# yikaiw/Vidu4D

Hardware: AMD Instinct MI355X
Metric: train images/sec (fwd+bwd raster) @200k surfels, 512^2 (higher is better)
Workload: dtype f32

## Files before the change

include/vidu4d_surfel.h:

```cpp
#ifndef VIDU4D_SURFEL_H_INCLUDED
#define VIDU4D_SURFEL_H_INCLUDED

#include <stddef.h>
#include <stdint.h>

#ifdef __cplusplus
extern "C" {
#endif

#define VIDU4D_OK 0
#define VIDU4D_E_INVALID (-1)
#define VIDU4D_E_BUFFER (-2)
#define VIDU4D_E_HIP (-3)
#define VIDU4D_E_UNSUPPORTED (-4)

#define VIDU4D_SURFEL_ABI 21
int vidu4d_surfel_abi_version(void);
const char* vidu4d_last_error(void);

size_t vidu4d_surfel_geom_bytes(int P);
size_t vidu4d_surfel_image_bytes(int width, int height);
size_t vidu4d_surfel_binning_bytes(int64_t capacity );
size_t vidu4d_surfel_backward_workspace_bytes(int P);

// ... 16 lines not shown
    const float* transMat_precomp;
    const float* viewmatrix;
    const float* projmatrix;
    const float* campos;
    float* out_color;
    float* out_others;
    int32_t* radii;
    void* geom_buffer;
    size_t geom_bytes;
    void* image_buffer;
    size_t image_bytes;
    int segment_split;
    uint32_t* depth_used;
    int frames;
    const float* frame_viewmatrix[8];
    const float* frame_campos[8];
    float frame_tan_fovx[8];
    float frame_tan_fovy[8];
    const float* sh_dc;
    const float* sh_rest;
    int raw_params;
    int aux_planes;
    int assume_unsaturated;
    int long_list_sort;
    int debug_flags;
    int max_list_hint;
} Vidu4dSurfelForwardArgs;
#define VIDU4D_AUX_ALPHA 0x02
#define VIDU4D_AUX_GEOM 0x1F
#define VIDU4D_DEBUG_NO_CULL 1
#define VIDU4D_DEBUG_WHOLE_TILE_BACKWARD 2
#define VIDU4D_DEBUG_POSITION_ORDER 8
#define VIDU4D_DEBUG_SERIAL_REPAIR 4
#define VIDU4D_SCHED_PAIR(K) (((K) & 15) << 12)
#define VIDU4D_SCHED_XCD_BLOCK(B) (((B) & 15) << 8)
#define VIDU4D_SURFEL_MAX_FRAMES 8
size_t vidu4d_surfel_image_bytes_frames(int width, int height, int frames);

int vidu4d_surfel_forward_plan(const Vidu4dSurfelForwardArgs* args, void* stream);
int vidu4d_surfel_num_rendered(const Vidu4dSurfelForwardArgs* args, void* stream, int64_t* num_rendered);
int vidu4d_surfel_forward_run(const Vidu4dSurfelForwardArgs* args, void* binning_buffer, size_t binning_bytes,
                              int64_t capacity, void* stream);

typedef struct Vidu4dSurfelBackwardArgs {
    int P, D, M;
    int width, height;
    float tan_fovx, tan_fovy;
    float scale_modifier;
    int debug;
    const float* background;
    const float* means3D;
    const int32_t* radii;
    const float* shs;
    const float* colors_precomp;
    const float* scales;
    const float* rotations;
    const float* transMat_precomp;
    const float* viewmatrix;
    const float* projmatrix;
    const float* campos;
    const float* dL_dout_color;
    const float* dL_dout_others;
    const void* geom_buffer;
    const void* binning_buffer;
    int64_t binning_capacity;
    const void* image_buffer;
// ... 248 lines not shown
```

vidu4d_amd/_C.py:

```python
from __future__ import annotations

import contextlib
import ctypes as C
import math
import os
import threading

import torch

from . import _lib

_EXACT = os.environ.get("VIDU4D_SURFEL_EXACT", "0") == "1"
_SPLIT = os.environ.get("VIDU4D_SURFEL_SPLIT", "auto")
SPLIT_AUTO_LEN = int(os.environ.get("VIDU4D_SURFEL_SPLIT_AUTO_LEN", "2048"))
SPLIT_AUTO_TILES_PER_CU = float(os.environ.get("VIDU4D_SURFEL_SPLIT_AUTO_TILES_PER_CU",
                                               "1.25" if int(os.environ.get("VIDU4D_SURFEL_PAIR", "6")) > 0 else "2.0"))
SEG_LEN = int(os.environ.get("VIDU4D_SEG_LEN", "512"))
MSD_SORT_FROM = int(os.environ.get("VIDU4D_MSD_SORT_FROM", "10000"))
_SPEC = os.environ.get("VIDU4D_SURFEL_SPEC", "1") == "1"
_SPEC_GEOM = os.environ.get("VIDU4D_SURFEL_SPEC_GEOM", "0") == "1"
DEBUG_FLAGS = ((_lib.DEBUG_NO_CULL if os.environ.get("VIDU4D_SURFEL_NO_CULL", "0") == "1" else 0) |
               (_lib.DEBUG_WHOLE_TILE_BACKWARD if os.environ.get("VIDU4D_SURFEL_WHOLE_TILE_BWD", "0") == "1" else 0) |
               (_lib.DEBUG_SERIAL_REPAIR if os.environ.get("VIDU4D_SURFEL_SERIAL_REPAIR", "0") == "1" else 0) |
               (_lib.DEBUG_POSITION_ORDER if os.environ.get("VIDU4D_SURFEL_POSITION_ORDER", "0") == "1" else 0))
XCD_BLOCK = int(os.environ.get("VIDU4D_SURFEL_XCD_BLOCK", "0"))
PAIR_K = int(os.environ.get("VIDU4D_SURFEL_PAIR", "6"))
_cu_count: dict = {}


class RasterContext:

    def __init__(self, scope=None):
        self.scope = scope
        self.deferred = False
        self.graph_mode = False
        self.graph_headers = None
        self.pending: list = []
        self.grad_out: dict = {}
        self.grad_written = None
        self.debug_flags = None
        self.xcd_block = None
        self.pair_k = None
        self.walk_counters = None
        self.capacity_hint: dict = {}
        self.depth_hint: dict = {}
        self.len_hint: dict = {}
        self.long_tiles_hint: dict = {}
        self.unlimited: dict = {}
        self.depth_stat: dict = {}
        self.pinned: dict = {}

    def __enter__(self):
        _stack().append(self)
        return self

    def __exit__(self, *exc):
        _stack().pop()
# ... 493 lines not shown
```

vidu4d_amd/_lib.py:

```python
from __future__ import annotations

import ctypes as C
import os

_HERE = os.path.dirname(os.path.abspath(__file__))
LIB_PATH = os.path.join(_HERE, "csrc", "libvidu4d_surfel.so")

ABI_VERSION = 21


class ForwardArgs(C.Structure):
    _fields_ = [
        ("P", C.c_int), ("D", C.c_int), ("M", C.c_int), ("width", C.c_int), ("height", C.c_int),
        ("tan_fovx", C.c_float), ("tan_fovy", C.c_float), ("scale_modifier", C.c_float),
        ("prefiltered", C.c_int), ("debug", C.c_int),
        ("background", C.c_void_p), ("means3D", C.c_void_p), ("shs", C.c_void_p), ("colors_precomp", C.c_void_p),
        ("opacities", C.c_void_p), ("scales", C.c_void_p), ("rotations", C.c_void_p),
        ("transMat_precomp", C.c_void_p), ("viewmatrix", C.c_void_p), ("projmatrix", C.c_void_p),
        ("campos", C.c_void_p), ("out_color", C.c_void_p), ("out_others", C.c_void_p), ("radii", C.c_void_p),
        ("geom_buffer", C.c_void_p), ("geom_bytes", C.c_size_t), ("image_buffer", C.c_void_p),
        ("image_bytes", C.c_size_t), ("segment_split", C.c_int), ("depth_used", C.c_void_p),
        ("frames", C.c_int), ("frame_viewmatrix", C.c_void_p * 8), ("frame_campos", C.c_void_p * 8),
        ("frame_tan_fovx", C.c_float * 8), ("frame_tan_fovy", C.c_float * 8),
        ("sh_dc", C.c_void_p), ("sh_rest", C.c_void_p), ("raw_params", C.c_int), ("aux_planes", C.c_int),
# ... 23 lines not shown
                ("src_v", C.c_void_p), ("dst_v", C.c_void_p), ("width", C.c_int)]


class SkinFieldArgs(C.Structure):
    _fields_ = [("N", C.c_int), ("B", C.c_int), ("W", C.c_int), ("D", C.c_int)] + [
        (n, C.c_void_p) for n in ("xyz", "bone_A", "bone_c", "w_in", "b_in", "w_hid", "b_hid", "w_out", "b_out", "xbT",
                                  "rawT", "g_xbT", "g_rawT", "g_xyz", "relu_masks", "packed_fwd", "packed_bwd", "h_store",
                                  "g_store", "gx_store")] + [("h_store_rows", C.c_int)]


LOSS_MAX_FRAMES, LOSS_BLOCKS, LOSS_SUMS_FLOATS = 32, 1024, 32


class Stage3LossArgs(C.Structure):
    _fields_ = [("M", C.c_int), ("H", C.c_int), ("W", C.c_int), ("color", C.c_void_p * LOSS_MAX_FRAMES),
                ("allmap", C.c_void_p * LOSS_MAX_FRAMES), ("bkgd", C.c_void_p), ("rgb", C.c_void_p),
                ("mask", C.c_void_p), ("vis2d", C.c_void_p), ("det", C.c_void_p), ("lambda_dssim", C.c_float),
                ("rgb_wt", C.c_float), ("mask_wt", C.c_float), ("dist_wt", C.c_float), ("sums", C.c_void_p),
                ("partials", C.c_void_p), ("losses", C.c_void_p), ("plane_stride", C.c_int64),
                ("normal_wt", C.c_float), ("depth_ratio", C.c_float), ("rays_d", C.c_void_p * LOSS_MAX_FRAMES),
                ("rays_o", C.c_void_p * LOSS_MAX_FRAMES), ("view3x3", C.c_void_p * LOSS_MAX_FRAMES),
                ("surf_normal", C.c_void_p * LOSS_MAX_FRAMES), ("surf_depth", C.c_void_p)]


class Stage3LossGrads(C.Structure):
    _fields_ = [("g_color", C.c_void_p * LOSS_MAX_FRAMES), ("g_allmap", C.c_void_p * LOSS_MAX_FRAMES),
                ("g_bkgd", C.c_void_p), ("g_surf_normal", C.c_void_p * LOSS_MAX_FRAMES)]


SKIN_FIELD = dict(width=64, in_max=96, out_max=32, max_hidden=4)
AUX_ALPHA = 0x02
AUX_GEOM = 0x1F
DEBUG_NO_CULL, DEBUG_WHOLE_TILE_BACKWARD, DEBUG_SERIAL_REPAIR, DEBUG_POSITION_ORDER = 1, 2, 4, 8



def sched_pair(k: int) -> int:
    return (int(k) & 15) << 12


def sched_xcd_block(block: int) -> int:
    return (int(block) & 15) << 8


BLEND_STATS = 11
ADAM_MAX_TENSORS = 8
ADAMW_MAX_TENSORS = 32
CONTRACT_MAX_JOBS = 4
COPY_MAX_JOBS = 8
CLIP_MAX_TENSORS = 96
CLIP_WORKSPACE_FLOATS = 1056
DENSIFY_MAX_ATTRS = 8


class BackwardArgs(C.Structure):
    _fields_ = [
        ("P", C.c_int), ("D", C.c_int), ("M", C.c_int), ("width", C.c_int), ("height", C.c_int),
        ("tan_fovx", C.c_float), ("tan_fovy", C.c_float), ("scale_modifier", C.c_float), ("debug", C.c_int),
        ("background", C.c_void_p), ("means3D", C.c_void_p), ("radii", C.c_void_p), ("shs", C.c_void_p),
        ("colors_precomp", C.c_void_p), ("scales", C.c_void_p), ("rotations", C.c_void_p),
        ("transMat_precomp", C.c_void_p), ("viewmatrix", C.c_void_p), ("projmatrix", C.c_void_p),
        ("campos", C.c_void_p), ("dL_dout_color", C.c_void_p), ("dL_dout_others", C.c_void_p),
        ("geom_buffer", C.c_void_p), ("binning_buffer", C.c_void_p), ("binning_capacity", C.c_int64),
        ("image_buffer", C.c_void_p), ("workspace", C.c_void_p), ("workspace_bytes", C.c_size_t),
        ("dL_dmeans2D", C.c_void_p), ("dL_dcolors", C.c_void_p), ("dL_dopacity", C.c_void_p),
        ("dL_dmeans3D", C.c_void_p), ("dL_dtransMat", C.c_void_p), ("dL_dsh", C.c_void_p),
# ... 123 lines not shown
```

vidu4d_amd/csrc/binning.hip:

```cpp
#include <algorithm>

#include "surfel_state.h"
#include "wave_utils.h"

namespace surfel {

__global__ __launch_bounds__(1024) void tile_scan_kernel(GeomState g, ImageState img, int num_tiles)
{
    __shared__ uint32_t s_part[16];
    const int lane = threadIdx.x & 63, wave = threadIdx.x >> 6;
    uint32_t carry = 0;
    for (int base = 0; base < num_tiles; base += 1024) {
        const int t = base + threadIdx.x;
        uint32_t cnt[TILE_SLICES];
        uint32_t c = 0;
        if (t < num_tiles) {
            const uint4* p = reinterpret_cast<const uint4*>(img.tile_count + (size_t)t * TILE_SLICES);
#pragma unroll
            for (int k = 0; k < TILE_SLICES / 4; k++) {
                const uint4 v = p[k];
                cnt[4 * k] = v.x;
                cnt[4 * k + 1] = v.y;
                cnt[4 * k + 2] = v.z;
                cnt[4 * k + 3] = v.w;
// ... 395 lines not shown
            const size_t b = (size_t)(tile0 + y * cam.grid_x + x) * TILE_SLICES + slice;
            const uint32_t pos = img.tile_base[b] + atomicAdd(&img.tile_count[b], 1u);
            entries[pos] = entry;
        }
}

template <bool COMPACT>
__global__ __launch_bounds__(BIN_THREADS) void emit_keys_grouped_kernel(CameraParams cam, int P, int iters,
                                                                       const int32_t* radii, GeomState g,
                                                                       ImageState img, uint64_t* entries,
                                                                       int64_t capacity, ScheduleParams sp)
{
    extern __shared__ __attribute__((aligned(16))) uint32_t s_cur[];
    if (blockIdx.x == gridDim.x - 1) {
        tile_order(g, img, cam.grid_x * cam.grid_y * cam.frames, *reinterpret_cast<TileOrderShared*>(s_cur), sp);
        return;
    }
    if (blockIdx.x == 0 && threadIdx.x == 0) g.hdr->num_buckets = 0;
    if ((int64_t)g.hdr->num_rendered > capacity) {
        if (blockIdx.x == 0 && threadIdx.x == 0) g.hdr->overflow = 1;
        return;
    }
    const int frame_tiles = cam.grid_x * cam.grid_y, num_tiles = frame_tiles * cam.frames;
    const uint32_t* row = img.group_counts + (size_t)blockIdx.x * num_tiles;
    for (int t = threadIdx.x; t < num_tiles; t += BIN_THREADS) s_cur[t] = img.ranges[2 * t] + row[t];
    __syncthreads();
    const int first = blockIdx.x * BIN_THREADS * iters;
    for (int it = 0; it < iters; it++) {
        const int idx = first + it * BIN_THREADS + threadIdx.x;
        if (idx >= P) continue;
        int radius;
        float cx, cy, depth;
        if (COMPACT) {
            const float4 c = reinterpret_cast<const float4*>(g.colour)[idx];
            cx = c.x, cy = c.y, depth = c.z, radius = __float_as_int(c.w);
            if (radius <= 0) continue;
        } else {
            radius = radii[idx];
            if (radius <= 0) continue;
            const float4 q2 = reinterpret_cast<const float4*>(g.rec + (size_t)idx * REC_FLOATS)[2];
            const float4 q3 = reinterpret_cast<const float4*>(g.rec + (size_t)idx * REC_FLOATS)[3];
            cx = q2.y, cy = q2.z, depth = q3.w;
        }
        int x0, y0, x1, y1;
        tile_rect(cx, cy, radius, cam.grid_x, cam.grid_y, x0, y0, x1, y1);
        const uint64_t entry = ((uint64_t)__float_as_uint(depth) << 32) | (uint32_t)idx;
        uint32_t* cur = s_cur + (cam.frames > 1 ? (idx / cam.frame_surfels) * frame_tiles : 0);
        for (int y = y0; y < y1; y++)
            for (int x = x0; x < x1; x++) entries[atomicAdd(&cur[y * cam.grid_x + x], 1u)] = entry;
    }
}

void launch_emit_keys(const CameraParams& cam, int P, const int32_t* radii, const GeomState& g, const ImageState& img,
                      const BinState& b, int64_t capacity, bool grouped, const ScheduleParams& sp, hipStream_t stream)
{
    if (P <= 0 || capacity <= 0) {
        launch_tile_order(g, img, total_tiles(cam), sp, stream);
        return;
    }
    if (grouped) {
        auto kernel = preprocess_stages_records(total_tiles(cam)) ? &emit_keys_grouped_kernel<true> : &emit_keys_grouped_kernel<false>;
        const size_t lds = std::max((size_t)total_tiles(cam) * sizeof(uint32_t), sizeof(TileOrderShared));
        hipLaunchKernelGGL(kernel, dim3(bin_groups(P) + 1), dim3(BIN_THREADS), lds, stream,
                           cam, P, bin_iters(P), radii, g, img, b.entries, capacity, sp);
    } else {
        launch_tile_order(g, img, total_tiles(cam), sp, stream);
        hipLaunchKernelGGL(emit_keys_kernel, dim3(pre_blocks(P)), dim3(PRE_BLOCK), 0, stream, cam, P, radii, g, img,
// ... 324 lines not shown
```

vidu4d_amd/csrc/capi.hip:

```cpp
#include <stdarg.h>
#include <stdio.h>
#include <string.h>

#include <vector>

#include "../../include/vidu4d_surfel.h"
#include "../../include/vidu4d_surfel_diag.h"
#include "surfel_state.h"

using namespace surfel;

static thread_local char g_err[512] = "";

static int fail(int code, const char* fmt, ...)
{
    va_list ap;
    va_start(ap, fmt);
    vsnprintf(g_err, sizeof(g_err), fmt, ap);
    va_end(ap);
    return code;
}

#define HIP_TRY(expr)                                                                                  \
    do {                                                                                               \
// ... 189 lines not shown
    if (int rc = check_frames(a)) return rc;
    if (F == 1 && (!(a->tan_fovx > 0.f) || !(a->tan_fovy > 0.f))) return fail(VIDU4D_E_INVALID, "tan_fov must be > 0");
    if (!a->out_color || !a->out_others || !a->background) return fail(VIDU4D_E_INVALID, "output/background pointer is NULL");
    if (a->P > 0 && (!a->means3D || !a->opacities || !a->scales || !a->rotations || !a->radii ||
                     (F == 1 && (!a->viewmatrix || !a->campos))))
        return fail(VIDU4D_E_INVALID, "an input pointer is NULL");
    if (!a->geom_buffer || a->geom_bytes < vidu4d_surfel_geom_bytes(a->P * F)) return fail(VIDU4D_E_BUFFER, "geom_buffer too small");
    if (!a->image_buffer || a->image_bytes < vidu4d_surfel_image_bytes_frames(a->width, a->height, F))
        return fail(VIDU4D_E_BUFFER, "image_buffer too small");
    return VIDU4D_OK;
}

__global__ __launch_bounds__(256) void zero_fill_kernel(uint4* p, size_t n16)
{
    const size_t i = (size_t)blockIdx.x * 256 + threadIdx.x;
    if (i < n16) p[i] = make_uint4(0u, 0u, 0u, 0u);
}
__global__ __launch_bounds__(256) void zero_fill_f32_kernel(float* p, size_t n)
{
    const size_t i = (size_t)blockIdx.x * 256 + threadIdx.x;
    if (i < n) p[i] = 0.f;
}
static void zero_fill_f32(float* p, size_t n, hipStream_t stream)
{
    if (n) hipLaunchKernelGGL(zero_fill_f32_kernel, dim3((unsigned)((n + 255) / 256)), dim3(256), 0, stream, p, n);
}
static void zero_fill(void* p, size_t bytes, hipStream_t stream)
{
    const size_t n16 = bytes / 16;
    if (n16)
        hipLaunchKernelGGL(zero_fill_kernel, dim3((unsigned)((n16 + 255) / 256)), dim3(256), 0, stream, (uint4*)p, n16);
}

extern "C" int vidu4d_surfel_forward_plan(const Vidu4dSurfelForwardArgs* a, void* stream_)
{
    hipStream_t stream = (hipStream_t)stream_;
    (void)hipGetLastError();
    int rc = check_forward(a);
    if (rc) return rc;
    GeomState g;
    ImageState img;
    const int F = frames_of(a), P = a->P * F;
    carve_geom((char*)a->geom_buffer, P, g);
    carve_image((char*)a->image_buffer, a->width, a->height, img, F);
    PreprocessArgs pa;
    pa.cam = camera_of(a);
    pa.P = P;
    pa.means3D = a->means3D;
    pa.scales = a->scales;
    pa.rotations = a->rotations;
    pa.opacities = a->opacities;
    pa.shs = a->shs;
    pa.colors_precomp = a->colors_precomp;
    pa.sh_dc = a->sh_dc;
    pa.sh_rest = a->sh_rest;
    pa.raw_params = a->raw_params;
    pa.radii = a->radii;
    pa.geom = g;
    pa.tile_count = img.tile_count;
    pa.group_counts = img.group_counts;
    pa.iters = bin_iters(P);
    pa.stage_records = 0;
    const int num_tiles = total_tiles(pa.cam);
    const bool grouped = use_grouped_binning(num_tiles);
    {
        StageTimer t(ST_PREPROCESS, stream);
        if (!grouped)
            zero_fill(img.tile_count, (size_t)num_tiles * TILE_SLICES * sizeof(uint32_t), stream);
        launch_preprocess_fwd(pa, stream);
    }
    STAGE_CHECK(a->debug, stream, "preprocess");
    {
        StageTimer t(ST_SCAN, stream);
        launch_tile_scan(g, img, num_tiles, grouped ? bin_groups(P) : 0, stream);
    }
    STAGE_CHECK(a->debug, stream, "tile_scan");
    return VIDU4D_OK;
}

extern "C" int vidu4d_surfel_num_rendered(const Vidu4dSurfelForwardArgs* a, void* stream_, int64_t* out)
{
    hipStream_t stream = (hipStream_t)stream_;
    if (!a || !out || !a->geom_buffer) return fail(VIDU4D_E_INVALID, "NULL argument");
    GeomState g;
    carve_geom((char*)a->geom_buffer, a->P * frames_of(a), g);
    uint32_t r = 0;
    HIP_TRY(hipMemcpyAsync(&r, &g.hdr->num_rendered, sizeof(r), hipMemcpyDeviceToHost, stream));
    HIP_TRY(hipStreamSynchronize(stream));
    *out = (int64_t)r;
    return VIDU4D_OK;
}

extern "C" int vidu4d_surfel_forward_run(const Vidu4dSurfelForwardArgs* a, void* binning, size_t binning_bytes,
                                         int64_t capacity, void* stream_)
{
    hipStream_t stream = (hipStream_t)stream_;
    (void)hipGetLastError();
    int rc = check_forward(a);
    if (rc) return rc;
    if (capacity < 0) return fail(VIDU4D_E_INVALID, "negative capacity");
    if (capacity > 0 && (!binning || binning_bytes < vidu4d_surfel_binning_bytes(capacity)))
        return fail(VIDU4D_E_BUFFER, "binning_buffer too small for capacity %lld", (long long)capacity);
    if (capacity > 0xFFFFFFFFll) return fail(VIDU4D_E_INVALID, "capacity exceeds the 32-bit pair index of the reference");
    GeomState g;
    ImageState img;
    BinState b;
    const int F = frames_of(a), P = a->P * F;
    carve_geom((char*)a->geom_buffer, P, g);
    carve_image((char*)a->image_buffer, a->width, a->height, img, F);
    carve_binning((char*)binning, capacity, b);
    const CameraParams cam = camera_of(a);
    const bool record = records_segments(a->segment_split, total_tiles(cam));
    const ScheduleParams sp = {record ? REC_SEG_LEN : SEG_LEN, record ? REC_MIN : SPLIT_MIN, 1,
                               (a->debug_flags >> FLAG_XCD_SHIFT) & 15, cam.grid_x, cam.grid_x * cam.grid_y,
                               (a->segment_split == 0 && !((a->debug_flags >> FLAG_XCD_SHIFT) & 15)) ? (a->debug_flags >> FLAG_PAIR_SHIFT) & 15 : 0};
    {
        StageTimer t(ST_EMIT, stream);
        launch_emit_keys(cam, P, a->radii, g, img, b, capacity, use_grouped_binning(total_tiles(cam)), sp, stream);
    }
    STAGE_CHECK(a->debug, stream, "emit_keys");
    if (capacity > 0) {
        {
            StageTimer t(ST_SORT, stream);
            launch_tile_sort(g, img, b, total_tiles(cam), P, capacity,
                             a->segment_split == 0 ? (a->max_list_hint > 0 && a->max_list_hint <= SHORT_LIST_HINT_MAX
                                                          ? LongListSort::short_lists_expected : LongListSort::in_lds_only)
                             : a->long_list_sort    ? LongListSort::one_workgroup
                                                    : LongListSort::msd_split,
                             stream);
        }
        STAGE_CHECK(a->debug, stream, "tile_sort");
    }
    {
        StageTimer t(ST_BLEND_FWD, stream);
        const int max_seg = a->segment_split > 1 ? a->segment_split : 0x7fffffff;
        launch_blend_fwd(cam, g, img, b, capacity, a->segment_split != 0, max_seg, a->background, a->out_color, a->out_others,
                         a->depth_used, blend_mode(a->aux_planes), a->assume_unsaturated != 0, kernel_flags(a->debug_flags),
                         record, stream);
    }
    STAGE_CHECK(a->debug, stream, "blend_forward");
    return VIDU4D_OK;
}

extern "C" int vidu4d_surfel_backward(const Vidu4dSurfelBackwardArgs* a, void* stream_)
{
    hipStream_t stream = (hipStream_t)stream_;
    (void)hipGetLastError();
    if (!a) return fail(VIDU4D_E_INVALID, "args is NULL");
    if (a->P < 0 || a->width <= 0 || a->height <= 0) return fail(VIDU4D_E_INVALID, "bad sizes");
    if (a->transMat_precomp) return fail(VIDU4D_E_UNSUPPORTED, "transMat_precomp is not supported (see forward)");
    if (a->P == 0) return VIDU4D_OK;
    const int F = frames_of(a), P = a->P * F;
    if (int rc = check_frames(a)) return rc;
    if (!a->geom_buffer || !a->image_buffer || !a->workspace || !a->dL_dout_color || !a->dL_dout_others ||
        !a->means3D || !a->radii || !a->scales || !a->rotations || (F == 1 && (!a->viewmatrix || !a->campos)) || !a->background)
        return fail(VIDU4D_E_INVALID, "an input pointer is NULL");
    if (!a->dL_dmeans2D || !a->dL_dcolors || !a->dL_dopacity || !a->dL_dmeans3D || !a->dL_dtransMat ||
        !a->dL_dscales || !a->dL_drotations || (a->shs && !a->dL_dsh))
        return fail(VIDU4D_E_INVALID, "an output pointer is NULL");
    if (int rc = check_canonical_sh(a)) return rc;
    if (a->sh_dc && (!a->dL_dsh_dc || !a->dL_dsh_rest || ((uintptr_t)a->dL_dsh_dc & 15) || ((uintptr_t)a->dL_dsh_rest & 15)))
        return fail(VIDU4D_E_INVALID, "sh_dc / sh_rest need 16-byte aligned dL_dsh_dc / dL_dsh_rest");
    if (a->workspace_bytes < vidu4d_surfel_backward_workspace_bytes(P)) return fail(VIDU4D_E_BUFFER, "workspace too small");
    if (a->binning_capacity > 0 && !a->binning_buffer) return fail(VIDU4D_E_INVALID, "binning_buffer is NULL");

// ... 135 lines not shown
```

vidu4d_amd/csrc/preprocess.hip:

```cpp
#include <cstdlib>

#include "surfel_state.h"
#include "wave_utils.h"

namespace surfel {

struct FrameIndex {
    int frame, shared;
};
__device__ __forceinline__ FrameIndex frame_index(const CameraParams& cam, int idx)
{
    if (cam.frames <= 1) return FrameIndex{0, idx};
    const int f = idx / cam.frame_surfels;
    return FrameIndex{f, idx - f * cam.frame_surfels};
}

__device__ __forceinline__ float act_scale(float raw) { return expf(raw); }
__device__ __forceinline__ float act_opacity(float raw) { return 1.0f / (1.0f + expf(-raw)); }

constexpr int SH_ROW = 48, SH_STRIDE = 49, SH_DC = 3, SH_REST = 45;

template <int WIDTH, int COL0>
__device__ __forceinline__ void tile_load_run(float* s_sh, const float* __restrict__ src, int rows)
{
// ... 44 lines not shown
{
    if (dL_dsh_dc) {
        tile_store_run<SH_DC, 0>(s_sh, dL_dsh_dc + (size_t)block_first * SH_DC, rows);
        tile_store_run<SH_REST, SH_DC>(s_sh, dL_dsh_rest + (size_t)block_first * SH_REST, rows);
    } else {
        tile_store_run<SH_ROW, 0>(s_sh, dL_dsh + (size_t)block_first * SH_ROW, rows);
    }
}

__device__ __forceinline__ uint32_t preprocess_one(const PreprocessArgs& a, const Camera& cam, int idx, int shared,
                                                   Projected& o, float4* stage = nullptr)
{
    const float p_world[3] = {a.means3D[3 * idx], a.means3D[3 * idx + 1], a.means3D[3 * idx + 2]};
    float2 sc = reinterpret_cast<const float2*>(a.scales)[shared];
    if (a.raw_params) sc = make_float2(act_scale(sc.x), act_scale(sc.y));
    const float4 q4 = reinterpret_cast<const float4*>(a.rotations)[idx];
    const float scale[2] = {sc.x, sc.y};
    const float quat[4] = {q4.x, q4.y, q4.z, q4.w};
    uint32_t tiles = 0;
    int radius = 0;
    if (project_surfel(cam, p_world, quat, scale, o)) {
        tiles = o.tiles;
        radius = o.radius;
        float4* rec = stage ? stage : reinterpret_cast<float4*>(a.geom.rec + (size_t)idx * REC_FLOATS);
        rec[0] = make_float4(o.T[0], o.T[1], o.T[2], o.T[3]);
        rec[1] = make_float4(o.T[4], o.T[5], o.T[6], o.T[7]);
        const float opacity = a.raw_params ? act_opacity(a.opacities[shared]) : a.opacities[shared];
        rec[2] = make_float4(o.T[8], o.center[0], o.center[1], opacity);
        rec[3] = make_float4(o.normal[0], o.normal[1], o.normal[2], o.depth);
        float f[8];
        contribution_footprint(o.T, o.center[0], o.center[1], opacity, f);
        rec[5] = make_float4(f[0], f[1], f[2], f[3]);
        rec[6] = make_float4(f[4], f[5], f[6], f[7]);
        if (stage) rec[4] = reinterpret_cast<const float4*>(a.geom.colour)[idx];
    }
    if (stage) reinterpret_cast<float4*>(a.geom.colour)[idx] =
        make_float4(o.center[0], o.center[1], o.depth, __int_as_float(radius));
    a.radii[idx] = radius;
    a.geom.tiles_touched[idx] = tiles;
    return tiles;
}

__device__ __forceinline__ void flush_staged_records(const float4* stage, float* rec, int idx0, unsigned long long visible,
                                                     int lane)
{
    __builtin_amdgcn_fence(__ATOMIC_RELEASE, "wavefront");
    __builtin_amdgcn_wave_barrier();
    __builtin_amdgcn_fence(__ATOMIC_ACQUIRE, "wavefront");
    if (visible) {
        float4* dst = reinterpret_cast<float4*>(rec + (size_t)idx0 * REC_FLOATS);
        constexpr int PARTS = REC_USED_FLOATS / 4, STRIDE = REC_FLOATS / 4;
#pragma unroll
        for (int i0 = 0; i0 < 64 * PARTS; i0 += 64) {
            const int i = i0 + lane, r = i / PARTS;
            if ((visible >> r) & 1ull) dst[PARTS == STRIDE ? i : r * STRIDE + (i - r * PARTS)] = stage[i];
        }
    }
    __builtin_amdgcn_fence(__ATOMIC_RELEASE, "wavefront");
    __builtin_amdgcn_wave_barrier();
}

__global__ __launch_bounds__(PRE_BLOCK) void preprocess_fwd_kernel(PreprocessArgs a)
{
    const int idx = blockIdx.x * PRE_BLOCK + threadIdx.x;
    if (idx == 0) {
        a.geom.hdr->min_T_bits = 0x3f800000u;
        a.geom.hdr->depth_used = 0;
    }
    if (idx >= a.P) return;
    const FrameIndex fi = frame_index(a.cam, idx);
// ... 45 lines not shown
    uint32_t* row = a.group_counts + (size_t)blockIdx.x * num_tiles;
    for (int t = threadIdx.x; t < num_tiles; t += BIN_THREADS) row[t] = s_hist[t];
}

template <bool SH_LDS>
__global__ __launch_bounds__(PRE_BLOCK) void surfel_color_kernel(PreprocessArgs a)
{
    extern __shared__ __attribute__((aligned(16))) float s_sh[];
    const int N = a.cam.frames > 1 ? a.cam.frame_surfels : a.P;
    const int block_first = blockIdx.x * PRE_BLOCK;
    const int shared = block_first + threadIdx.x;
    const int rows = (N - block_first) < PRE_BLOCK ? (N - block_first) : PRE_BLOCK;
    if (SH_LDS) {
        sh_tile_load(s_sh, a.shs, a.sh_dc, a.sh_rest, block_first, rows);
        __syncthreads();
    }
    if (shared >= N) return;
    const int F = a.cam.frames > 1 ? a.cam.frames : 1;
    for (int frame = 0; frame < F; frame++) {
        const int idx = frame * N + shared;
        float rgb[3];
        uint32_t clamp_mask = 0;
        if (a.colors_precomp == nullptr) {
            const float p_world[3] = {a.means3D[3 * idx], a.means3D[3 * idx + 1], a.means3D[3 * idx + 2]};
            const float* cp = a.cam.fc[frame].campos;
            const float campos[3] = {cp[0], cp[1], cp[2]};
            const float* sh = SH_LDS ? s_sh + threadIdx.x * SH_STRIDE : a.shs + (size_t)shared * a.cam.sh_coeffs * 3;
            sh_forward(a.cam.sh_degree, p_world, campos, sh, rgb, clamp_mask);
        } else {
            rgb[0] = a.colors_precomp[3 * idx];
            rgb[1] = a.colors_precomp[3 * idx + 1];
            rgb[2] = a.colors_precomp[3 * idx + 2];
        }
        float4* dst = a.stage_records ? reinterpret_cast<float4*>(a.geom.colour) + idx
                                      : reinterpret_cast<float4*>(a.geom.rec + (size_t)idx * REC_FLOATS) + 4;
        *dst = make_float4(rgb[0], rgb[1], rgb[2], __uint_as_float(clamp_mask));
    }
}

static bool stage_records_enabled();
bool preprocess_stages_records(int num_tiles)
{
    static int big_lds = -1;
    if (big_lds < 0)
        big_lds = hipFuncSetAttribute(reinterpret_cast<const void*>(&preprocess_fwd_grouped_kernel),
                                      hipFuncAttributeMaxDynamicSharedMemorySize, 160 * 1024) == hipSuccess;
    const size_t hist = (size_t)((num_tiles + 3) & ~3) * sizeof(uint32_t);
    const size_t staged = hist + (size_t)(BIN_THREADS / 64) * 64 * REC_USED_FLOATS * sizeof(float);
    return use_grouped_binning(num_tiles) && big_lds == 1 && staged <= 160 * 1024 && stage_records_enabled();
}

static bool stage_records_enabled()
{
    static int v = -1;
    if (v < 0) {
        const char* e = getenv("VIDU4D_STAGE_RECORDS");
        v = e ? atoi(e) : 1;
    }
    return v != 0;
}

void launch_preprocess_fwd(const PreprocessArgs& a, hipStream_t stream)
{
    if (a.P <= 0) return;
    const int num_tiles = total_tiles(a.cam);
    const bool sh_lds = a.colors_precomp == nullptr && a.cam.sh_coeffs == 16 &&
                        (a.sh_dc != nullptr || (a.shs != nullptr && (reinterpret_cast<uintptr_t>(a.shs) & 15) == 0));
    const int color_blocks = a.cam.frames > 1 ? pre_blocks(a.cam.frame_surfels) : pre_blocks(a.P);
    PreprocessArgs g = a;
    g.stage_records = 0;
    const size_t hist = (size_t)((num_tiles + 3) & ~3) * sizeof(uint32_t);
    const size_t staged = hist + (size_t)(BIN_THREADS / 64) * 64 * REC_USED_FLOATS * sizeof(float);
    g.stage_records = preprocess_stages_records(num_tiles) ? 1 : 0;
    if (sh_lds)
        hipLaunchKernelGGL(surfel_color_kernel<true>, dim3(color_blocks), dim3(PRE_BLOCK),
                           (size_t)PRE_BLOCK * SH_STRIDE * sizeof(float), stream, g);
    else
        hipLaunchKernelGGL(surfel_color_kernel<false>, dim3(color_blocks), dim3(PRE_BLOCK), 0, stream, g);
    if (use_grouped_binning(num_tiles))
        hipLaunchKernelGGL(preprocess_fwd_grouped_kernel, dim3(bin_groups(a.P)), dim3(BIN_THREADS),
                           g.stage_records ? staged : hist, stream, g);
    else
        hipLaunchKernelGGL(preprocess_fwd_kernel, dim3(pre_blocks(a.P)), dim3(PRE_BLOCK), 0, stream, a);
}


template <bool SH_LDS>
__global__ __launch_bounds__(PRE_BLOCK) void preprocess_bwd_kernel(BackwardArgs a)
{
    extern __shared__ __attribute__((aligned(16))) float s_sh[];
    const bool stacked = a.cam.frames > 1;
    const int N = stacked ? a.cam.frame_surfels : a.P;
    const int per_frame = pre_blocks(N);
    const int frame = blockIdx.x / per_frame;
    const int block_first = (blockIdx.x - frame * per_frame) * PRE_BLOCK;
    const int shared = block_first + threadIdx.x;
    const int idx = frame * N + shared;
    const Camera cam = load_camera(a.cam, frame);
    const int M = cam.sh_coeffs;
    const int rows = (N - block_first) < PRE_BLOCK ? (N - block_first) : PRE_BLOCK;
    if (SH_LDS) {
        sh_tile_load(s_sh, a.shs, a.sh_dc, a.sh_rest, block_first, rows);
        __syncthreads();
    }
    const bool has_sh = a.shs != nullptr || a.sh_dc != nullptr;
    const bool live = shared < N;
    const bool visible = live && a.radii[idx] > 0;
    float* sh_row = s_sh + threadIdx.x * SH_STRIDE;
    float* dsh = (a.dL_dsh && live) ? a.dL_dsh + (size_t)shared * M * 3 : nullptr;
    if (live && !visible) {
        for (int k = 0; k < 3; k++) {
// ... 241 lines not shown
```

vidu4d_amd/csrc/surfel_state.h:

```cpp
#pragma once

#include <hip/hip_runtime.h>
#include <stddef.h>
#include <stdint.h>

#include "surfel_math.h"

namespace surfel {

constexpr int PRE_BLOCK = 256;
constexpr int TILE_SLICES = 16;
constexpr int BIN_THREADS = 1024;
#ifndef SURFEL_BIN_MAX_GROUPS
#define SURFEL_BIN_MAX_GROUPS 256
#endif
constexpr int BIN_MAX_GROUPS = SURFEL_BIN_MAX_GROUPS;
constexpr int BIN_MAX_TILES = 16384;
constexpr int TILE_SORT_CAP = 3584;

#ifndef SURFEL_SEG_LEN
#define SURFEL_SEG_LEN 512
#endif
#ifndef SURFEL_SPLIT_MIN
#define SURFEL_SPLIT_MIN 1024
// ... 48 lines not shown
constexpr int FLAG_XCD_SHIFT = 8;
constexpr int FLAG_POSITION_ORDER = 8;
constexpr int FLAG_PAIR_SHIFT = 12;
constexpr int PAIR_MAX = 1024;
constexpr int FLAG_SERIAL_REPAIR = 4;

struct Header {
    uint32_t num_rendered;
    uint32_t overflow;
    uint32_t max_tile_len;
    uint32_t num_segments;
    uint32_t num_split_pos;
    uint32_t split_used;
    uint32_t truncated;
    uint32_t scan_arrivals;
    uint32_t min_T_bits;
    uint32_t num_buckets;
    uint32_t seg_len;
    uint32_t split_min;
    uint32_t depth_used;
    uint32_t num_live_full;
    uint32_t num_long_tiles;
    uint32_t xcd_block;
    uint32_t live_xcd;
    uint32_t num_paired;
    uint32_t pad[46];
};
static_assert(sizeof(Header) == 256, "the header is the first 256 bytes of the geometry buffer");

struct GeomState {
    Header* hdr;
    float* rec;
    uint32_t* tiles_touched;
    float* colour;
};

struct ImageState {
    float* final_T;
    uint32_t* n_contrib;
    uint32_t* ranges;
    uint32_t* tile_count;
    uint32_t* tile_base;
    uint32_t* group_counts;
    uint32_t* tile_order;
    uint32_t* seg_first;
    uint32_t* seg_prefix;
    uint32_t* tail_order;
    float* tile_m0;
    uint32_t* live_count;
    uint32_t* live_prefix;
};

struct BinState {
    uint64_t* entries;
    uint64_t* scratch;
    uint32_t* point_list;
    float* seg_data;
};

template <typename T>
inline void carve(char*& p, T*& out, size_t count)
{
    uintptr_t a = (reinterpret_cast<uintptr_t>(p) + 255) & ~uintptr_t(255);
    out = reinterpret_cast<T*>(a);
    p = reinterpret_cast<char*>(out + count);
}

__host__ __device__ inline int pre_blocks(int P) { return (P + PRE_BLOCK - 1) / PRE_BLOCK; }
inline int bin_iters(int P)
{
    const long long per = (long long)BIN_THREADS * BIN_MAX_GROUPS;
    const int k = (int)((P + per - 1) / per);
    return k > 1 ? k : 1;
}
inline int bin_groups(int P) { const int sb = BIN_THREADS * bin_iters(P); return (P + sb - 1) / sb; }
inline bool use_grouped_binning(int num_tiles) { return num_tiles <= BIN_MAX_TILES; }

inline size_t carve_geom(char* base, int P, GeomState& g)
{
    char* p = base;
    carve(p, g.hdr, 1);
    carve(p, g.rec, (size_t)P * REC_FLOATS);
    carve(p, g.tiles_touched, (size_t)P);
    carve(p, g.colour, (size_t)P * 4);
    return (size_t)(p - base) + 256;
}

inline size_t carve_image(char* base, int W, int H, ImageState& s, int frames = 1)
{
    char* p = base;
    const size_t hw = (size_t)W * H * frames;
    const size_t tiles = (size_t)((W + TILE - 1) / TILE) * ((H + TILE - 1) / TILE) * frames;
    carve(p, s.final_T, 3 * hw);
    carve(p, s.n_contrib, 2 * hw);
    carve(p, s.ranges, 2 * tiles);
    carve(p, s.tile_count, tiles * TILE_SLICES);
    carve(p, s.tile_base, tiles * TILE_SLICES);
    carve(p, s.group_counts, tiles <= (size_t)BIN_MAX_TILES ? tiles * BIN_MAX_GROUPS : 0);
    carve(p, s.tile_order, tiles);
    carve(p, s.seg_first, tiles);
    carve(p, s.seg_prefix, tiles + 1);
    carve(p, s.tail_order, tiles);
    carve(p, s.tile_m0, tiles);
    carve(p, s.live_count, tiles);
    carve(p, s.live_prefix, tiles + 1);
    return (size_t)(p - base) + 256;
}

inline size_t carve_binning(char* base, int64_t capacity, BinState& b)
{
    char* p = base;
    const size_t cap = (size_t)(capacity > 0 ? capacity : 0);
    carve(p, b.entries, cap);
    carve(p, b.scratch, cap);
    carve(p, b.point_list, cap);
    carve(p, b.seg_data, cap ? seg_data_floats(capacity) : 0);
    return (size_t)(p - base) + 256;
// ... 59 lines not shown
    c.cy = p.cy;
    c.tan_fovx = fc.tan_fovx;
    c.tan_fovy = fc.tan_fovy;
    c.W = p.W;
    c.H = p.H;
    c.grid_x = p.grid_x;
    c.grid_y = p.grid_y;
    c.sh_degree = p.sh_degree;
    c.sh_coeffs = p.sh_coeffs;
    return c;
}
#endif

struct PreprocessArgs {
    CameraParams cam;
    int P;
    const float* means3D;
    const float* scales;
    const float* rotations;
    const float* opacities;
    const float* shs;
    const float* colors_precomp;
    const float* sh_dc;
    const float* sh_rest;
    int raw_params;
    int32_t* radii;
    GeomState geom;
    uint32_t* tile_count;
    uint32_t* group_counts;
    int iters;
    int stage_records;
};
void launch_preprocess_fwd(const PreprocessArgs& a, hipStream_t stream);
void launch_tile_scan(const GeomState& g, const ImageState& img, int num_tiles, int groups, hipStream_t stream);
struct ScheduleParams {
    int seg_len, split_min, by_class;
    int xcd_block, grid_x, frame_tiles;
    int pair_k;
};
void launch_tile_order(const GeomState& g, const ImageState& img, int num_tiles, const ScheduleParams& sp, hipStream_t stream);
void launch_emit_keys(const CameraParams& cam, int P, const int32_t* radii, const GeomState& g, const ImageState& img,
                      const BinState& b, int64_t capacity, bool grouped, const ScheduleParams& sp, hipStream_t stream);
enum class LongListSort { in_lds_only, msd_split, one_workgroup, short_lists_expected };
constexpr int SHORT_LIST_HINT_MAX = 900;
bool preprocess_stages_records(int num_tiles);
void launch_tile_sort(const GeomState& g, const ImageState& img, const BinState& b, int num_tiles, int num_surfels,
                      int64_t capacity, LongListSort mode, hipStream_t stream);
void launch_blend_fwd(const CameraParams& cam, const GeomState& g, const ImageState& img, const BinState& b,
                      int64_t capacity, bool split, int max_seg, const float* background, float* out_color,
                      float* out_others, uint32_t* depth_used, int mode, bool assume_unsaturated, int flags, bool record,
                      hipStream_t stream);

struct BackwardArgs {
    CameraParams cam;
    int P;
    const float* background;
    const float* means3D;
    const int32_t* radii;
    const float* shs;
    const float* colors_precomp;
    const float* scales;
    const float* rotations;
    const float* dL_dcolor;
    const float* dL_dothers;
    GeomState geom;
    ImageState img;
// ... 34 lines not shown
```

Baseline: 3042.

## Run SH colour evaluation on a side stream overlapping binning and sort

Moves the surfel colour (SH evaluation) kernel out of the preprocess launch and runs it on a low-priority side stream, forked after planning and joined just before forward blending. The colour now always goes straight into the per-surfel record instead of being staged through a shared colour buffer, and that buffer is repurposed as a dedicated centre array used by key emission. This lets colour work overlap emit-keys, scan and tile sort, at the cost of extra events, a per-thread per-device stream, and possible contention for CUs. A debug flag restores serial execution.

After: 3054 (median of 6 runs). About the same (+0.4%).

```diff
diff --git a/include/vidu4d_surfel.h b/include/vidu4d_surfel.h
--- a/include/vidu4d_surfel.h
+++ b/include/vidu4d_surfel.h
@@ -72,6 +72,7 @@
 #define VIDU4D_DEBUG_WHOLE_TILE_BACKWARD 2
 #define VIDU4D_DEBUG_POSITION_ORDER 8
 #define VIDU4D_DEBUG_SERIAL_REPAIR 4
+#define VIDU4D_DEBUG_SERIAL_COLOUR 16
 #define VIDU4D_SCHED_PAIR(K) (((K) & 15) << 12)
 #define VIDU4D_SCHED_XCD_BLOCK(B) (((B) & 15) << 8)
 #define VIDU4D_SURFEL_MAX_FRAMES 8
diff --git a/vidu4d_amd/_C.py b/vidu4d_amd/_C.py
--- a/vidu4d_amd/_C.py
+++ b/vidu4d_amd/_C.py
@@ -22,7 +22,8 @@
 DEBUG_FLAGS = ((_lib.DEBUG_NO_CULL if os.environ.get("VIDU4D_SURFEL_NO_CULL", "0") == "1" else 0) |
                (_lib.DEBUG_WHOLE_TILE_BACKWARD if os.environ.get("VIDU4D_SURFEL_WHOLE_TILE_BWD", "0") == "1" else 0) |
                (_lib.DEBUG_SERIAL_REPAIR if os.environ.get("VIDU4D_SURFEL_SERIAL_REPAIR", "0") == "1" else 0) |
-               (_lib.DEBUG_POSITION_ORDER if os.environ.get("VIDU4D_SURFEL_POSITION_ORDER", "0") == "1" else 0))
+               (_lib.DEBUG_POSITION_ORDER if os.environ.get("VIDU4D_SURFEL_POSITION_ORDER", "0") == "1" else 0) |
+               (_lib.DEBUG_SERIAL_COLOUR if os.environ.get("VIDU4D_SURFEL_SERIAL_COLOUR", "0") == "1" else 0))
 XCD_BLOCK = int(os.environ.get("VIDU4D_SURFEL_XCD_BLOCK", "0"))
 PAIR_K = int(os.environ.get("VIDU4D_SURFEL_PAIR", "6"))
 _cu_count: dict = {}
diff --git a/vidu4d_amd/_lib.py b/vidu4d_amd/_lib.py
--- a/vidu4d_amd/_lib.py
+++ b/vidu4d_amd/_lib.py
@@ -79,6 +79,7 @@
 AUX_ALPHA = 0x02
 AUX_GEOM = 0x1F
 DEBUG_NO_CULL, DEBUG_WHOLE_TILE_BACKWARD, DEBUG_SERIAL_REPAIR, DEBUG_POSITION_ORDER = 1, 2, 4, 8
+DEBUG_SERIAL_COLOUR = 16
 
 
 
diff --git a/vidu4d_amd/csrc/binning.hip b/vidu4d_amd/csrc/binning.hip
--- a/vidu4d_amd/csrc/binning.hip
+++ b/vidu4d_amd/csrc/binning.hip
@@ -451,7 +451,7 @@
         int radius;
         float cx, cy, depth;
         if (COMPACT) {
-            const float4 c = reinterpret_cast<const float4*>(g.colour)[idx];
+            const float4 c = g.centre[idx];
             cx = c.x, cy = c.y, depth = c.z, radius = __float_as_int(c.w);
             if (radius <= 0) continue;
         } else {
diff --git a/vidu4d_amd/csrc/capi.hip b/vidu4d_amd/csrc/capi.hip
--- a/vidu4d_amd/csrc/capi.hip
+++ b/vidu4d_amd/csrc/capi.hip
@@ -245,17 +245,43 @@
         hipLaunchKernelGGL(zero_fill_kernel, dim3((unsigned)((n16 + 255) / 256)), dim3(256), 0, stream, (uint4*)p, n16);
 }
 
-extern "C" int vidu4d_surfel_forward_plan(const Vidu4dSurfelForwardArgs* a, void* stream_)
-{
-    hipStream_t stream = (hipStream_t)stream_;
-    (void)hipGetLastError();
-    int rc = check_forward(a);
-    if (rc) return rc;
-    GeomState g;
-    ImageState img;
-    const int F = frames_of(a), P = a->P * F;
-    carve_geom((char*)a->geom_buffer, P, g);
-    carve_image((char*)a->image_buffer, a->width, a->height, img, F);
+struct SideStream {
+    hipStream_t stream = nullptr;
+    hipEvent_t fork = nullptr, join = nullptr;
+};
+constexpr int MAX_SIDE_DEVICES = 64;
+static thread_local SideStream t_side[MAX_SIDE_DEVICES];
+
+static int side_stream(hipStream_t caller, SideStream** out)
+{
+    int dev = 0;
+    HIP_TRY(hipStreamGetDevice(caller, &dev));
+    if (dev < 0 || dev >= MAX_SIDE_DEVICES) return fail(VIDU4D_E_INVALID, "device %d out of range", dev);
+    SideStream& s = t_side[dev];
+    if (!s.stream) {
+        int cur = 0;
+        HIP_TRY(hipGetDevice(&cur));
+        HIP_TRY(hipSetDevice(dev));
+        int least = 0, greatest = 0;
+        hipError_t e = hipDeviceGetStreamPriorityRange(&least, &greatest);
+        if (e == hipSuccess) e = hipStreamCreateWithPriority(&s.stream, hipStreamNonBlocking, least);
+        if (e == hipSuccess) e = hipEventCreateWithFlags(&s.fork, hipEventDisableTiming);
+        if (e == hipSuccess) e = hipEventCreateWithFlags(&s.join, hipEventDisableTiming);
+        (void)hipSetDevice(cur);
+        if (e != hipSuccess) {
+            if (s.join) (void)hipEventDestroy(s.join);
+            if (s.fork) (void)hipEventDestroy(s.fork);
+            if (s.stream) (void)hipStreamDestroy(s.stream);
+            s = SideStream();
+            return fail(VIDU4D_E_HIP, "side stream: %s", hipGetErrorString(e));
+        }
+    }
+    *out = &s;
+    return VIDU4D_OK;
+}
+
+static PreprocessArgs preprocess_args(const Vidu4dSurfelForwardArgs* a, const GeomState& g, const ImageState& img, int P)
+{
     PreprocessArgs pa;
     pa.cam = camera_of(a);
     pa.P = P;
@@ -274,6 +300,21 @@
     pa.group_counts = img.group_counts;
     pa.iters = bin_iters(P);
     pa.stage_records = 0;
+    return pa;
+}
+
+extern "C" int vidu4d_surfel_forward_plan(const Vidu4dSurfelForwardArgs* a, void* stream_)
+{
+    hipStream_t stream = (hipStream_t)stream_;
+    (void)hipGetLastError();
+    int rc = check_forward(a);
+    if (rc) return rc;
+    GeomState g;
+    ImageState img;
+    const int F = frames_of(a), P = a->P * F;
+    carve_geom((char*)a->geom_buffer, P, g);
+    carve_image((char*)a->image_buffer, a->width, a->height, img, F);
+    const PreprocessArgs pa = preprocess_args(a, g, img, P);
     const int num_tiles = total_tiles(pa.cam);
     const bool grouped = use_grouped_binning(num_tiles);
     {
@@ -324,6 +365,16 @@
     carve_binning((char*)binning, capacity, b);
     const CameraParams cam = camera_of(a);
     const bool record = records_segments(a->segment_split, total_tiles(cam));
+    SideStream* side = nullptr;
+    if (!a->debug && !(a->debug_flags & VIDU4D_DEBUG_SERIAL_COLOUR))
+        if (int rc2 = side_stream(stream, &side)) return rc2;
+    if (side) {
+        HIP_TRY(hipEventRecord(side->fork, stream));
+        HIP_TRY(hipStreamWaitEvent(side->stream, side->fork, 0));
+    }
+    launch_surfel_color(preprocess_args(a, g, img, P), side ? side->stream : stream);
+    if (side) HIP_TRY(hipEventRecord(side->join, side->stream));
+    STAGE_CHECK(a->debug, stream, "surfel_color");
     const ScheduleParams sp = {record ? REC_SEG_LEN : SEG_LEN, record ? REC_MIN : SPLIT_MIN, 1,
                                (a->debug_flags >> FLAG_XCD_SHIFT) & 15, cam.grid_x, cam.grid_x * cam.grid_y,
                                (a->segment_split == 0 && !((a->debug_flags >> FLAG_XCD_SHIFT) & 15)) ? (a->debug_flags >> FLAG_PAIR_SHIFT) & 15 : 0};
@@ -344,6 +395,7 @@
         }
         STAGE_CHECK(a->debug, stream, "tile_sort");
     }
+    if (side) HIP_TRY(hipStreamWaitEvent(stream, side->join, 0));
     {
         StageTimer t(ST_BLEND_FWD, stream);
         const int max_seg = a->segment_split > 1 ? a->segment_split : 0x7fffffff;
diff --git a/vidu4d_amd/csrc/preprocess.hip b/vidu4d_amd/csrc/preprocess.hip
--- a/vidu4d_amd/csrc/preprocess.hip
+++ b/vidu4d_amd/csrc/preprocess.hip
@@ -100,10 +100,8 @@
         contribution_footprint(o.T, o.center[0], o.center[1], opacity, f);
         rec[5] = make_float4(f[0], f[1], f[2], f[3]);
         rec[6] = make_float4(f[4], f[5], f[6], f[7]);
-        if (stage) rec[4] = reinterpret_cast<const float4*>(a.geom.colour)[idx];
-    }
-    if (stage) reinterpret_cast<float4*>(a.geom.colour)[idx] =
-        make_float4(o.center[0], o.center[1], o.depth, __int_as_float(radius));
+    }
+    if (stage) a.geom.centre[idx] = make_float4(o.center[0], o.center[1], o.depth, __int_as_float(radius));
     a.radii[idx] = radius;
     a.geom.tiles_touched[idx] = tiles;
     return tiles;
@@ -215,9 +213,8 @@
             rgb[1] = a.colors_precomp[3 * idx + 1];
             rgb[2] = a.colors_precomp[3 * idx + 2];
         }
-        float4* dst = a.stage_records ? reinterpret_cast<float4*>(a.geom.colour) + idx
-                                      : reinterpret_cast<float4*>(a.geom.rec + (size_t)idx * REC_FLOATS) + 4;
-        *dst = make_float4(rgb[0], rgb[1], rgb[2], __uint_as_float(clamp_mask));
+        reinterpret_cast<float4*>(a.geom.rec + (size_t)idx * REC_FLOATS)[4] = make_float4(rgb[0], rgb[1], rgb[2],
+                                                                                            __uint_as_float(clamp_mask));
     }
 }
 
@@ -243,23 +240,27 @@
     return v != 0;
 }
 
-void launch_preprocess_fwd(const PreprocessArgs& a, hipStream_t stream)
+void launch_surfel_color(const PreprocessArgs& a, hipStream_t stream)
 {
     if (a.P <= 0) return;
-    const int num_tiles = total_tiles(a.cam);
     const bool sh_lds = a.colors_precomp == nullptr && a.cam.sh_coeffs == 16 &&
                         (a.sh_dc != nullptr || (a.shs != nullptr && (reinterpret_cast<uintptr_t>(a.shs) & 15) == 0));
     const int color_blocks = a.cam.frames > 1 ? pre_blocks(a.cam.frame_surfels) : pre_blocks(a.P);
+    if (sh_lds)
+        hipLaunchKernelGGL(surfel_color_kernel<true>, dim3(color_blocks), dim3(PRE_BLOCK),
+                           (size_t)PRE_BLOCK * SH_STRIDE * sizeof(float), stream, a);
+    else
+        hipLaunchKernelGGL(surfel_color_kernel<false>, dim3(color_blocks), dim3(PRE_BLOCK), 0, stream, a);
+}
+
+void launch_preprocess_fwd(const PreprocessArgs& a, hipStream_t stream)
+{
+    if (a.P <= 0) return;
+    const int num_tiles = total_tiles(a.cam);
     PreprocessArgs g = a;
-    g.stage_records = 0;
     const size_t hist = (size_t)((num_tiles + 3) & ~3) * sizeof(uint32_t);
     const size_t staged = hist + (size_t)(BIN_THREADS / 64) * 64 * REC_USED_FLOATS * sizeof(float);
     g.stage_records = preprocess_stages_records(num_tiles) ? 1 : 0;
-    if (sh_lds)
-        hipLaunchKernelGGL(surfel_color_kernel<true>, dim3(color_blocks), dim3(PRE_BLOCK),
-                           (size_t)PRE_BLOCK * SH_STRIDE * sizeof(float), stream, g);
-    else
-        hipLaunchKernelGGL(surfel_color_kernel<false>, dim3(color_blocks), dim3(PRE_BLOCK), 0, stream, g);
     if (use_grouped_binning(num_tiles))
         hipLaunchKernelGGL(preprocess_fwd_grouped_kernel, dim3(bin_groups(a.P)), dim3(BIN_THREADS),
                            g.stage_records ? staged : hist, stream, g);
diff --git a/vidu4d_amd/csrc/surfel_state.h b/vidu4d_amd/csrc/surfel_state.h
--- a/vidu4d_amd/csrc/surfel_state.h
+++ b/vidu4d_amd/csrc/surfel_state.h
@@ -104,7 +104,7 @@
     Header* hdr;
     float* rec;
     uint32_t* tiles_touched;
-    float* colour;
+    float4* centre;
 };
 
 struct ImageState {
@@ -154,7 +154,7 @@
     carve(p, g.hdr, 1);
     carve(p, g.rec, (size_t)P * REC_FLOATS);
     carve(p, g.tiles_touched, (size_t)P);
-    carve(p, g.colour, (size_t)P * 4);
+    carve(p, g.centre, (size_t)P);
     return (size_t)(p - base) + 256;
 }
 
@@ -280,6 +280,7 @@
     int stage_records;
 };
 void launch_preprocess_fwd(const PreprocessArgs& a, hipStream_t stream);
+void launch_surfel_color(const PreprocessArgs& a, hipStream_t stream);
 void launch_tile_scan(const GeomState& g, const ImageState& img, int num_tiles, int groups, hipStream_t stream);
 struct ScheduleParams {
     int seg_len, split_min, by_class;
```
